# fryzjergda/DesiRNA

Hardware: AMD Instinct MI355X
Metric: replica-folds/sec (MFE+PF, L=200, R=64) (higher is better)
Workload: dtype int32 (MFE) + f64 (PF); 1 GPU; BASELINE configs[2]: Eterna100-V1 #69 target (L=200), R=64 uniform-random sequences per GPU, -sf Ed-Epf (MFE fill+traceback, PF inside, eval_structure); replicas_per_gpu=64, replicas_total=64, replicas_on_rank0=64, L=200, exchange_every=100, threads_per_workgroup=1024

## Files before the change

desirna_amd/csrc/fold_pf_lds.hpp:

```cpp
#pragma once
#include <cstddef>
#include "eval_structure.hpp"
#include "fold_pf.hpp"

namespace drna {

constexpr int PF_FAST_NMAX = 200;
constexpr int PGSLOTS = 10;
constexpr int PNG = 3;
constexpr int TSL = 14;

template <int NT>
struct PfFastSmem {
  static constexpr int NW = NT / WAVE;
  static constexpr int RS = PF_FAST_NMAX + 2;
  static constexpr int NSLOT = 4 * WAVE;
  static constexpr int NL = PF_FAST_NMAX + 8;
  double qbi[32 * RS];
  double dring[4 * RS];
  double qm1row[2][RS];
  double urow[2][RS];
  double hpw[PF_FAST_NMAX + 2];
  double q5[PF_FAST_NMAX + 2];
  double partG[2][2][NSLOT];
  double partK[2][4][NSLOT];
  double accE[2][NSLOT], accX[2][3][NSLOT];
  double stack[64], mmH[128], mmI[128], mm1n[128], mm23[128], mmM[128], mmExt[128], int11[1024], d5[32], d3[32];
  double rinv[128];
  double rbul[128];
  double r1n[128];
  double r23[128];
  double eWt[36][2];
  double xc[16];
  double twc[32][2];
  int plist[2][NL];
  int pcnt[2];
  int qhead[2];
  int qtile[2];
  unsigned char info[32 * RS];
  unsigned char S[PF_FAST_NMAX + 4];
  int flag;
};

template <int NT>
__device__ __forceinline__ void pf_q5_column(PfFastSmem<NT>& sm, const double* __restrict__ QEXT, int ld, int j, int lane,
                                             double sc1) {
  double s = 0.0;
  for (int i = lane + 1; i <= j - TURN - 1; i += WAVE) s += sm.q5[i - 1] * QEXT[j * ld + i];
  s = wave_total_f64_lane63(s);
  if (lane == WAVE - 1) sm.q5[j] = sm.q5[j - 1] * sc1 + s;
  wave_lds_sync();
}

template <class SM>
__device__ __forceinline__ void pf_prepare_tables(SM& sm, int d, int tid) {
  constexpr int RS = SM::RS;
  if (tid >= 0 && tid < GRES) {
    const int par = d & 1;
    const int x = (int)((unsigned)(d + 50 - tid) % (unsigned)GRES);
    const int zero_row = 32 * RS * 8;
    int offA = zero_row, offB = zero_row;
    double eas = 0.0, keep = 1.0, W = 0.0;
    if (x <= 26) {
      const int s = x + 4, dp = d - 6 - x;
      if (dp <= TURN) keep = 0.0;
      else {
        const int base = (dp & 31) * RS * 8;
        offA = base + 3 * 8;
        offB = s == 4 ? zero_row : base + (s - 1) * 8;
        eas = sm.tw_as[s];
        keep = s <= 5 ? 0.0 : 1.0;
        W = sm.tw_W[s];
      }
    }
    sm.tw_i[par][tid][0] = offA; sm.tw_i[par][tid][1] = offB;
    sm.tw_d[par][tid][0] = eas; sm.tw_d[par][tid][1] = keep; sm.tw_d[par][tid][2] = W;
  }
}

__device__ __forceinline__ double lane_table_f64(double v, int l) {
  return __hiloint2double(__builtin_amdgcn_readlane(__double2hiint(v), l), __builtin_amdgcn_readlane(__double2loint(v), l));
}

template <class SM, int R0, int R1>
__device__ __forceinline__ double pf_tower_part(const SM& sm, double (&G)[PGSLOTS], int i8, int eA, int eB, double eas,
                                                double ekeep, double eW) {
  const char* ring = reinterpret_cast<const char*>(sm.qbi);
  double a[R1 - R0], b[R1 - R0];
#pragma unroll
  for (int r = R0; r < R1; r++) {
    a[r - R0] = *reinterpret_cast<const double*>(ring + lane_table(eA, r) + i8);
    b[r - R0] = *reinterpret_cast<const double*>(ring + lane_table(eB, r) + i8);
  }
  double acc = 0.0;
#pragma unroll
  for (int r = R0; r < R1; r++) {
    G[r] = G[r] * lane_table_f64(ekeep, r) + (a[r - R0] + b[r - R0]) * lane_table_f64(eas, r);
    acc += G[r] * lane_table_f64(eW, r);
  }
  return acc;
}

template <class SM>
__device__ __forceinline__ double pf_tower_step(const SM& sm, double (&G)[PGSLOTS], int par, int i8, int g, int lane) {
  const int rr = lane * PNG + g;
  const bool on = lane < PGSLOTS && rr < GRES;
  const int zero_row = 32 * SM::RS * 8;
  const int eA = on ? sm.tw_i[par][rr][0] : zero_row, eB = on ? sm.tw_i[par][rr][1] : zero_row;
  const double eas = on ? sm.tw_d[par][rr][0] : 0.0, ekeep = on ? sm.tw_d[par][rr][1] : 1.0, eW = on ? sm.tw_d[par][rr][2] : 0.0;
  const double lo = pf_tower_part<SM, 0, PGSLOTS / 2>(sm, G, i8, eA, eB, eas, ekeep, eW);
  const double hi = pf_tower_part<SM, PGSLOTS / 2, PGSLOTS>(sm, G, i8, eA, eB, eas, ekeep, eW);
  return lo + hi;
}


template <class SM, int SIG, int Q0, int Q1>
__device__ __forceinline__ void pf_tower2_part(const SM& sm, double (&G)[TSL], int dv, int i8, int cbase, double& acc) {
  const char* ring = reinterpret_cast<const char*>(sm.qbi);
  double a[Q1 - Q0], b[Q1 - Q0];
  f64x2 c[Q1 - Q0];
#pragma unroll
  for (int q = Q1 - 1; q >= Q0; q--) {
    const int s = 4 + SIG + 2 * q;
    if (s > 30) continue;
    const int va = ((dv - s) & 31) * (SM::RS * 8) + i8;
    a[q - Q0] = *reinterpret_cast<const double*>(ring + va + 24);
    b[q - Q0] = s == 4 ? 0.0 : *reinterpret_cast<const double*>(ring + va + (s - 1) * 8);
    c[q - Q0] = *reinterpret_cast<const f64x2*>(ring + cbase + s * 16);
  }
#pragma unroll
  for (int q = Q1 - 1; q >= Q0; q--) {
    const int s = 4 + SIG + 2 * q;
    if (s > 30) continue;
    G[q] = q > 0 ? fma3_f64(a[q - Q0] + b[q - Q0], c[q - Q0].x, G[q - 1]) : (a[q - Q0] + b[q - Q0]) * c[q - Q0].x;
    acc += G[q] * c[q - Q0].y;
  }
}

template <class SM, int SIG>
__device__ __forceinline__ double pf_tower2_step(const SM& sm, double (&G)[TSL], int dv, int i8) {
  const int cbase = as_vector((int)(reinterpret_cast<const char*>(&sm.twc[0][0]) - reinterpret_cast<const char*>(sm.qbi)));
  double acc0 = 0.0, acc1 = 0.0, acc2 = 0.0;
  pf_tower2_part<SM, SIG, 9, 14>(sm, G, dv, i8, cbase, acc0);
  pf_tower2_part<SM, SIG, 4, 9>(sm, G, dv, i8, cbase, acc1);
  pf_tower2_part<SM, SIG, 0, 4>(sm, G, dv, i8, cbase, acc2);
  return (acc0 + acc1) + acc2;
}


#ifndef DRNA_PKE
#define DRNA_PKE 5
#endif
constexpr int PKE = DRNA_PKE;
constexpr int KT_NL = PKE + 3;
constexpr int KT_U = (2 * KT_NL + 3) / 4;
constexpr int KT_BMIN = (12 + 2 * PKE + 3) / 4;
constexpr int KT_D0 = 4 * KT_BMIN - 3;
constexpr int KT_MF = (4 * ((PF_FAST_NMAX - 1) / 4) - 11 - 2 * PKE + 15) / 16;
constexpr int KT_DEPTH = 3;
static_assert(PKE >= 4, "a tile's operands must be final when the first of its four steps comes");

__device__ __forceinline__ void kt_near_counts(int i, int d, int& nl, int& nh) {
  const int j = i + d, a = (i - 1) >> 2, c = (j - 1) >> 2, tot = max(d - 2 * TURN - 2, 0);
  if (c - a >= KT_BMIN) { nl = 4 * a + 4 + PKE - i; nh = j - 4 * c - 1 + PKE; }
  else { nl = min(tot, KT_NL); nh = tot - nl; }
}
__device__ __forceinline__ bool kt_has_far(int i, int d) { return ((i + d - 1) >> 2) - ((i - 1) >> 2) >= KT_BMIN; }

template <typename RS>
__device__ __forceinline__ void k_near_row(RS rs, int tab8, int ld, int d, int i, int row, double& v0, double& v1) {
  int nl0, nh0, nl1, nh1;
  kt_near_counts(i, d, nl0, nh0);
  kt_near_counts(i + 1, d, nl1, nh1);
  f64x2 a[KT_U], c[KT_U];
#pragma unroll
  for (int u = 0; u < KT_U; u++) {
    const int s = row + 4 * u, y = s - KT_NL;
    const bool low = s < KT_NL;
    const bool ok0 = low ? s < nl0 : y < nh0, ok1 = low ? s < nl1 : y < nh1;
    int tt = low ? TURN + 1 + s : d - TURN - 2 - y;
    tt = (ok0 || ok1) ? tt : TURN + 1;
    a[u] = buf_load_f64x2(rs, (tt * ld + i) * 8, 0);
    c[u] = buf_load_f64x2(rs, tab8 + ((d - tt - 1) * ld + i + tt + 1) * 8, 0);
    if (!ok0) a[u].x = 0.0;
    if (!ok1) a[u].y = 0.0;
  }
  double p0 = 0.0, p1 = 0.0, q0 = 0.0, q1 = 0.0;
#pragma unroll
  for (int u = 0; u < KT_U; u++) {
    if (u & 1) { p1 = fma(a[u].x, c[u].x, p1); q1 = fma(a[u].y, c[u].y, q1); }
    else { p0 = fma(a[u].x, c[u].x, p0); q0 = fma(a[u].y, c[u].y, q0); }
  }
  v0 = p0 + p1; v1 = q0 + q1;
}

constexpr int KT_PRE = 3;
struct KTile {
  double al, bl, av[KT_PRE], bv[KT_PRE];
  int vA, vB;
  int a, c, last;
  bool mask_last;
};
template <bool SC1, typename RS>
__device__ __forceinline__ void k_tile_issue(RS rs, int tab8, int ld, int n, int a, int B, int lane, KTile& t) {
  const int c = a + B, m_lo = 4 * a + 9 + PKE, m_hi = 4 * c - 3 - PKE;
  const int last = __builtin_amdgcn_readfirstlane((m_hi - m_lo + 16) >> 4) - 1;
  const int q = lane & 3, moff = (lane & 12) + (lane >> 4);
  const int i = 4 * a + 1 + q, jc = min(4 * c + 1 + q, n);
  const int sA = 16 * ld * 8, sB = 16 * (ld - 1) * 8;
  const int m0 = m_lo + moff, ml = min(m0 + 16 * last, m_hi);
  const int vA = (i - (1 + i) * ld + m0 * ld) * 8;
  const int vB = tab8 + (jc * ld - (m0 + 16 * last) * (ld - 1)) * 8;
  const int vAl = (i - (1 + i) * ld + ml * ld) * 8, vBl = tab8 + (jc * ld - ml * (ld - 1)) * 8;
  t.a = a; t.c = c; t.last = last; t.mask_last = m0 + 16 * last > m_hi; t.vA = vA; t.vB = vB;
#pragma unroll
  for (int u = 0; u < KT_PRE; u++) {
    if (u < last) {
      t.av[u] = SC1 ? buf_load_f64_aux(rs, vA, u * sA) : buf_load_f64(rs, vA, u * sA);
      t.bv[u] = SC1 ? buf_load_f64_aux(rs, vB, (last - u) * sB) : buf_load_f64(rs, vB, (last - u) * sB);
    }
  }
  t.al = SC1 ? buf_load_f64_aux(rs, vAl, 0) : buf_load_f64(rs, vAl, 0);
  t.bl = SC1 ? buf_load_f64_aux(rs, vBl, 0) : buf_load_f64(rs, vBl, 0);
}
template <bool SC1, typename RS, typename ST>
__device__ __forceinline__ void k_tile_finish(RS rs, int ld, const KTile& t, int n, int lane, ST store) {
  const int sA = 16 * ld * 8, sB = 16 * (ld - 1) * 8, last = t.last;
  double acc0 = 0.0, acc1 = 0.0;
#pragma unroll
  for (int u = 0; u < KT_PRE; u++) {
    if (u < last) {
      if (u & 1) acc1 = mfma_f64_4x4x4_4b(t.av[u], t.bv[u], acc1);
      else acc0 = mfma_f64_4x4x4_4b(t.av[u], t.bv[u], acc0);
    }
  }
#pragma unroll
  for (int u0 = KT_PRE; u0 < KT_MF - 1; u0 += KT_DEPTH) {
    if (u0 < last) {
      double av[KT_DEPTH], bv[KT_DEPTH];
#pragma unroll
      for (int w = 0; w < KT_DEPTH; w++) {
        const int u = u0 + w;
        if (u < last && u < KT_MF - 1) {
          av[w] = SC1 ? buf_load_f64_aux(rs, t.vA, u * sA) : buf_load_f64(rs, t.vA, u * sA);
          bv[w] = SC1 ? buf_load_f64_aux(rs, t.vB, (last - u) * sB) : buf_load_f64(rs, t.vB, (last - u) * sB);
        }
      }
#pragma unroll
      for (int w = 0; w < KT_DEPTH; w++) {
        const int u = u0 + w;
        if (u < last && u < KT_MF - 1) {
          if (u & 1) acc1 = mfma_f64_4x4x4_4b(av[w], bv[w], acc1);
          else acc0 = mfma_f64_4x4x4_4b(av[w], bv[w], acc0);
        }
      }
    }
  }
  const double al = t.mask_last ? 0.0 : t.al;
  if (last & 1) acc1 = mfma_f64_4x4x4_4b(al, t.bl, acc1);
  else acc0 = mfma_f64_4x4x4_4b(al, t.bl, acc0);
  double v = acc0 + acc1;
  v = dpp_add_f64<0x114, 0xF>(v);
  v = dpp_add_f64<0x118, 0xF>(v);
  const int ii = 4 * t.a + 1 + (lane >> 4), jj = 4 * t.c + 1 + (lane & 3);
  if ((lane & 12) == 12 && jj <= n) store(jj - ii, ii, v);
}

#ifndef DRNA_PFL_D1
#define DRNA_PFL_D1 24
#endif
constexpr int PFL_D1 = DRNA_PFL_D1;
template <bool AGENT, class SM>
__device__ __forceinline__ void pf_pl_row(const SM& sm, int32_t* PL, int ld, int n, int d, int lane) {
  int cntb = 0;
  for (int i0 = 1; i0 <= n - d; i0 += WAVE) {
    const int i = i0 + lane;
    int t = 0;
    if (i <= n - d) t = pair_type(sm.S[i], sm.S[i + d]);
    const unsigned long long m = __ballot(t != 0);
    if (t) {
      const int pos = cntb + __popcll(m & ((1ull << lane) - 1ull));
      const int32_t w = i | ((t * 16 + sm.S[i + 1] * 4 + sm.S[i + d - 1]) << 8);
      if (AGENT) st_agent(&PL[d * ld + pos], w); else PL[d * ld + pos] = w;
    }
    cntb += __popcll(m);
  }
  if (lane == 0) { if (AGENT) st_agent(&PL[d * ld + ld - 1], (int32_t)cntb); else PL[d * ld + ld - 1] = cntb; }
}

template <int NT>
__device__ __forceinline__ void pf_kfar_helper(const PfArgs& A, const EvalArgs& EV, PfFastSmem<NT>& sm, int r, int n) {
  constexpr int NW = NT / WAVE;
  const int ld = A.ld, tid = threadIdx.x, lane = lane_id();
  const int wave = __builtin_amdgcn_readfirstlane(wave_id());
  double* base = A.ws + (long long)r * A.ws_stride;
  const long long tab = (long long)ld * ld;
  double* DFAR = base + 5 * tab;
  const auto rsX = __builtin_amdgcn_make_buffer_rsrc((void*)base, (short)0, (int)(2 * tab * 8), 0x00020000);
  const int* flagA = A.hflags + (long long)r * 64;
  int* flagB = A.hflags + (long long)r * 64 + 32;
  int* ctl = reinterpret_cast<int*>(&sm);
  if (tid == 0) ctl[0] = 0;
  if (EV.n_targets > 0) {
    constexpr int NEV = NW < 8 ? NW : 8;
    EvalSmem* es = reinterpret_cast<EvalSmem*>(ctl + 32);
    if (wave < NEV)
      for (int k = wave; k < EV.n_targets; k += NEV) eval_one(es[wave], EV, r, k, lane);
  }
  {
    const char* seq = A.seqs + A.rg.off_of(r, n);
    for (int k = tid; k < n; k += NT) { const int c = enc_nt(seq[k]); sm.S[k + 1] = (unsigned char)(c < 0 ? 0 : c); }
    if (tid == 0) { sm.S[0] = 0; sm.S[n + 1] = 0; }
    __syncthreads();
    int32_t* PL = reinterpret_cast<int32_t*>(base + 4 * tab);
    for (int d = PFL_D1 + wave; d < n; d += NW) pf_pl_row<true>(sm, PL, ld, n, d, lane);
    drain_vmem();
  }
  __syncthreads();
  if (tid == 0) st_agent(flagB, A.hbase + KT_D0 - 1);
  const int Bmax = (n - 1) >> 2;
  for (int B = KT_BMIN; B <= Bmax; B++) {
    if (wave == 0) {
      int seen = 0;
      const bool ok = strip_wait(flagA, A.hbase, 4 * B - 5 - PKE, seen);
      if (lane == 0 && (!ok || seen == A.hbase + STRIP_DONE)) ctl[0] = 1;
    }
    __syncthreads();
    if (ctl[0]) break;
    if (!(DRNA_SKIP & 8))
      for (int a = wave; a <= Bmax - B; a += NW) {
        KTile t;
        k_tile_issue<true>(rsX, (int)tab * 8, ld, n, a, B, lane, t);
        k_tile_finish<true>(rsX, ld, t, n, lane, [&](int d, int i, double v) { st_agent(&DFAR[d * ld + i], v); });
      }
    drain_vmem();
    __syncthreads();
    if (tid == 0) st_agent(flagB, A.hbase + (B == Bmax ? n : 4 * B));
  }
}

template <int NT, bool TILES = true>
__device__ __forceinline__ void pf_lds_body(PfFastSmem<NT>& sm, PfArgs A, const EvalArgs& EV, int bx_in = -1, int helper_in = -1) {
  constexpr int NW = NT / WAVE;
  constexpr int RS = PfFastSmem<NT>::RS;
  const PfTables& T = *A.T;
  const bool hm = A.helper != 0;
  const int bx = bx_in >= 0 ? bx_in : hm ? blockIdx.x >> 1 : blockIdx.x;
  const bool is_helper = hm && (helper_in >= 0 ? helper_in != 0 : (blockIdx.x & 1) != 0);
  const int r = A.rg.seq_of(bx);
  A.L = A.rg.len_of(r, A.L);
  const int n = A.L, ld = A.ld;
  if (is_helper) {
    if (A.helper == 2) return;
    pf_kfar_helper<NT>(A, EV, sm, r, n);
    return;
  }
  const int tid = threadIdx.x, lane = lane_id();
  const int wave = __builtin_amdgcn_readfirstlane(wave_id());

  double* base = A.ws + (long long)r * A.ws_stride;
  const long long tab = (long long)ld * ld;
  double* QM = base + 2 * tab;
  double* QM1 = base + 3 * tab;
  int32_t* PL = reinterpret_cast<int32_t*>(base + 4 * tab);
  double* QEXT = base + 6 * tab;

  const double eTau = T.TermAU, eMLc = T.MLclosing, eMLi = T.MLintern;
  const double b1 = A.eMLb[1], sc1 = A.scale[1], sc2 = A.scale[2];

  stage_energy_tables<NT>(sm, T, tid);
  for (int k = tid; k < 128; k += NT) {
    const double inv = 1.0 / T.mmI[k];
    sm.rinv[k] = inv;
    sm.rbul[k] = ((k >> 4) > 2 ? eTau : 1.0) * inv;
    sm.r1n[k] = T.mm1n[k] * inv;
    sm.r23[k] = T.mm23[k] * inv;
  }
  for (int k = tid; k <= n; k += NT) sm.hpw[k] = A.hp_w[k];
  for (int t = tid; t < 36; t += NT) {
    sm.eWt[t][0] = t >= 2 && t <= 30 ? T.bulge[t] * A.scale[t + 2] : 0.0;
    sm.eWt[t][1] = t >= 4 && t <= 30 ? T.interior[t] * T.eninio[t - 2] * A.scale[t + 2] : 0.0;
  }
  if (tid == 0) {
    sm.xc[0] = T.bulge[1] * A.scale[3]; sm.xc[1] = T.interior[5] * T.eninio[1] * A.scale[7];
    sm.xc[2] = A.scale[4]; sm.xc[3] = A.scale[5]; sm.xc[4] = A.scale[6];
    sm.xc[8] = eTau; sm.xc[9] = eMLc; sm.xc[10] = eMLi; sm.xc[11] = b1; sm.xc[12] = sc2;
  }
  for (int k = tid; k < 32; k += NT) {
    sm.twc[k][0] = k >= 4 && k <= 30 ? T.eninio[k - 4] : 0.0;
    sm.twc[k][1] = k >= 6 && k <= 30 ? T.interior[k] * A.scale[k + 2] : 0.0;
  }
  for (int k = tid; k < 4 * RS; k += NT) sm.dring[k] = 0.0;
  for (int k = tid; k < 32 * RS; k += NT) { sm.qbi[k] = 0.0; sm.info[k] = 0; }
  for (int k = tid; k < 2 * RS; k += NT) { (&sm.qm1row[0][0])[k] = 0.0; (&sm.urow[0][0])[k] = 0.0; }
  for (int k = tid; k < 2 * 2 * PfFastSmem<NT>::NSLOT; k += NT) (&sm.partG[0][0][0])[k] = 0.0;
  for (int k = tid; k < 2 * 4 * PfFastSmem<NT>::NSLOT; k += NT) (&sm.partK[0][0][0])[k] = 0.0;
  for (int k = tid; k < 2 * PfFastSmem<NT>::NSLOT; k += NT) (&sm.accE[0][0])[k] = 0.0;
  for (int k = tid; k < 6 * PfFastSmem<NT>::NSLOT; k += NT) (&sm.accX[0][0][0])[k] = 0.0;
  if (tid == 0) sm.q5[0] = 1.0;
  load_sequence<NT>(sm, A.seqs + A.rg.off_of(r, n), n, tid);
  if (sm.flag) {
    if (tid == 0) { A.status[r] = ST_BAD_CHAR; A.Epf[r] = 0.0; if (hm) st_agent(A.hflags + (long long)r * 64, A.hbase + STRIP_DONE); }
    return;
  }
  if (wave == 0) {
    for (int j = 1; j <= n && j <= TURN + 1; j++) sm.q5[j] = sm.q5[j - 1] * sc1;
  }
  for (int d = TURN + 1 + wave; d < (hm ? min(n, PFL_D1) : n); d += NW) pf_pl_row<false>(sm, PL, ld, n, d, lane);
  __syncthreads();

  const int NB = (n + WAVE - 1) / WAVE;
  const int off0 = (NB * WAVE - n) / 2;
  const int aw = wave - NB;
  constexpr bool TWO_PAR = NT < 1024;
  const int nT = n - 10, NBT = nT > 0 ? (nT + WAVE - 1) / WAVE : 0;
  const int T0 = max(0, off0 + 5 - (NBT * WAVE - nT) / 2);
  int my_tb = -1, my_sig = 0, my_pm = 0;
  if (aw >= 0) {
    if (TWO_PAR) { if (aw < 2 * NBT) { my_tb = aw >> 1; my_sig = aw & 1; my_pm = 3; } }
    else if (aw < 4 * NBT) { my_tb = aw >> 2; const int x = (aw + my_tb) & 3; my_sig = x & 1; my_pm = 1 << (x >> 1); }
  }
  const int w_pl = NB > 2 ? 2 : 0, w_q5 = NB - 1;

  if (aw < 0) {
    const int d = TURN + 1;
    if (d < n) {
      const int cnt = PL[d * ld + ld - 1];
      if (tid < cnt) sm.plist[d & 1][tid] = PL[d * ld + tid];
      if (tid == 0) { sm.pcnt[d & 1] = cnt; sm.qhead[0] = 0; sm.qhead[1] = 0; sm.qtile[0] = 0; sm.qtile[1] = 0; }
    }
  }
  __syncthreads();


  const auto rsQ = __builtin_amdgcn_make_buffer_rsrc((void*)QM, (short)0, (int)(2 * tab * 8), 0x00020000);


  double* XQM = base, *XQM1 = base + tab, *DFAR = base + 5 * tab;
  int* flagA = hm ? A.hflags + (long long)r * 64 : nullptr;
  const int* flagB = hm ? A.hflags + (long long)r * 64 + 32 : nullptr;
  double dfar_cur = 0.0, dfar_next = 0.0;
  int fb_last = 0;
  bool helper_lost = false, pl_seen = false;
  auto run_items = [&](const int d) {
    const int ncell = n - d, sh = d >> 1, par = d & 1;
    const int slot0 = sh + off0 - 1;
    const int pcnt = __builtin_amdgcn_readfirstlane(sm.pcnt[par]);
    const int nblk = (ncell + 31) >> 5;
    const int nK = ((DRNA_SKIP & 8) || d < 2 * TURN + 3) ? 0 : nblk;
    const int nE = (DRNA_SKIP & 2) ? 0 : (pcnt + 3) >> 2, nX = (DRNA_SKIP & 4) ? 0 : 3 * ((pcnt + WAVE - 1) / WAVE);
    const int nItems = __builtin_amdgcn_readfirstlane(nK + nE + nX);
    for (int it0 = queue_pop(&sm.qhead[par], lane); it0 < nItems; it0 = queue_pop(&sm.qhead[par], lane)) {
      const int it = it0 < nX ? nK + nE + it0 : it0 - nX;
      if (it < nK) {
        const int blk = it, cl = lane & 15, row = lane >> 4;
        int i = (blk << 5) + 2 * cl + 1;
        const bool act0 = i <= ncell, act1 = i + 1 <= ncell;
        i = act0 ? i : 1;
        double v0, v1;
        k_near_row(rsQ, (int)tab * 8, ld, d, i, row, v0, v1);
        if (act0) sm.partK[par][row][i + slot0] = v0;
        if (act1) sm.partK[par][row][i + 1 + slot0] = v1;
      } else if (it < nK + nE) {
        const int q = 4 * (it - nK) + (lane >> 4);
        const int pe = sm.plist[par][q < pcnt ? q : pcnt - 1];
        const int i0 = pe & 255, ij = pe >> 8;
        const int tA = (lane & 15) + 2, tBr = tA + 16, tB = tBr > 30 ? 30 : tBr;
        const f64x2 wA = *reinterpret_cast<const f64x2*>(&sm.eWt[tA][0]), wB = *reinterpret_cast<const f64x2*>(&sm.eWt[tBr][0]);
        const int oA = ((d - 2 - tA) & 31) * RS + i0, oB = ((d - 2 - tB) & 31) * RS + i0;
        const double a1 = sm.qbi[oA + 1], a2 = sm.qbi[oA + 2], a3 = sm.qbi[oA + tA], a4 = sm.qbi[oA + tA + 1];
        const double b1_ = sm.qbi[oB + 1], b2_ = sm.qbi[oB + 2], b3_ = sm.qbi[oB + tB], b4_ = sm.qbi[oB + tB + 1];
        const int fa1 = sm.info[oA + 1], fa2 = sm.info[oA + 2], fa3 = sm.info[oA + tA], fa4 = sm.info[oA + tA + 1];
        const int fb1 = sm.info[oB + 1], fb2 = sm.info[oB + 2], fb3 = sm.info[oB + tB], fb4 = sm.info[oB + tB + 1];
        const double ra1 = sm.rbul[fa1], ra4 = sm.rbul[fa4], ra2 = sm.r1n[fa2], ra3 = sm.r1n[fa3];
        const double rb1 = sm.rbul[fb1], rb4 = sm.rbul[fb4], rb2 = sm.r1n[fb2], rb3 = sm.r1n[fb3];
        const double bul = (a1 * ra1 + a4 * ra4) * wA.x + (b1_ * rb1 + b4_ * rb4) * wB.x;
        const double one = (a2 * ra2 + a3 * ra3) * wA.y + (b2_ * rb2 + b3_ * rb3) * wB.y;
        double v = bul * ((ij >> 4) > 2 ? sm.xc[as_vector(8)] : 1.0) + one * sm.mm1n[ij];
        v = dpp_add_f64<0x111, 0xF>(v);
        v = dpp_add_f64<0x112, 0xF>(v);
        v = dpp_add_f64<0x114, 0xF>(v);
        v = dpp_add_f64<0x118, 0xF>(v);
        if ((lane & 15) == 15 && q < pcnt) sm.accE[par][i0 + slot0] = v;
      } else {
        const int xi = it - nK - nE;
        const int ch = xi / 3, grp = xi - 3 * ch;
        const int q = ch * WAVE + lane;
        const int pe = sm.plist[par][q < pcnt ? q : pcnt - 1];
        const int i = pe & 255, cxv = pe >> 8, t = cxv >> 4, si1 = (cxv >> 2) & 3, sj1 = cxv & 3;
        double sum;
        if (grp == 0) {
          double w[4];
          int f[4];
#pragma unroll
          for (int shp = 0; shp < 4; shp++) {
            const int u1 = shp >> 1, u2 = shp == 1 || shp == 3 ? 1 : 0;
            const int dp = d - 2 - u1 - u2;
            const int off = (dp & 31) * RS + 1 + u1 + i;
            w[shp] = dp > TURN ? sm.qbi[off] : 0.0;
            f[shp] = dp > TURN ? sm.info[off] : 0;
          }
          sum = w[0] * sm.rinv[f[0]] * sm.stack[t * 8 + (f[0] >> 4)] * sm.xc[as_vector(12)];
          sum += (w[1] * sm.rinv[f[1]] * sm.stack[t * 8 + (f[1] >> 4)] + w[2] * sm.rinv[f[2]] * sm.stack[t * 8 + (f[2] >> 4)]) * sm.xc[as_vector(0)];
          sum += w[3] * sm.rinv[f[3]] * sm.int11[(t * 8 + (f[3] >> 4)) * 16 + si1 * 4 + sj1] * sm.xc[as_vector(2)];
        } else if (grp == 1) {
          const int dpa = d - 5, dpb = d - 6;
          const int oa = (dpa & 31) * RS + 2 + i, ob = (dpa & 31) * RS + 3 + i, oc = (dpb & 31) * RS + 3 + i;
          const double wa = dpa > TURN ? sm.qbi[oa] : 0.0, wb = dpa > TURN ? sm.qbi[ob] : 0.0, wc = dpb > TURN ? sm.qbi[oc] : 0.0;
          const int fa = dpa > TURN ? sm.info[oa] : 0, fb = dpa > TURN ? sm.info[ob] : 0, fc = dpb > TURN ? sm.info[oc] : 0;
          const double ga = T.int21[(t * 8 + (fa >> 4)) * 64 + si1 * 16 + ((fa >> 2) & 3) * 4 + sj1];
          const double gb = T.int21[((fb >> 4) * 8 + t) * 64 + ((fb >> 2) & 3) * 16 + si1 * 4 + (fb & 3)];
          const double gc = T.int22[(t * 8 + (fc >> 4)) * 256 + si1 * 64 + (fc & 3) * 16 + ((fc >> 2) & 3) * 4 + sj1];
          sum = (wa * sm.rinv[fa] * ga + wb * sm.rinv[fb] * gb) * sm.xc[as_vector(3)] + wc * sm.rinv[fc] * gc * sm.xc[as_vector(4)];
        } else {
          const int dp = d - 7;
          const int oa = (dp & 31) * RS + 3 + i, ob = (dp & 31) * RS + 4 + i;
          const double wa = dp > TURN ? sm.qbi[oa] : 0.0, wb = dp > TURN ? sm.qbi[ob] : 0.0;
          const int fa = dp > TURN ? sm.info[oa] : 0, fb = dp > TURN ? sm.info[ob] : 0;
          sum = (wa * sm.r23[fa] + wb * sm.r23[fb]) * sm.mm23[cxv] * sm.xc[as_vector(1)];
        }
        if (q < pcnt) sm.accX[par][grp][i + slot0] = sum;
      }
    }
  };

  auto run_tiles = [&](const int d) {
    const int Bmax = (n - 1) >> 2, Bt = ((d + 3) >> 2) + 1, ph = (d + 3) & 3;
    if (!TILES || (DRNA_SKIP & 8) || hm || Bt < KT_BMIN || Bt > Bmax) return;
    const int cnt = Bmax - Bt + 1, per = (cnt + 3) >> 2, a0 = ph * per;
    const int nT = __builtin_amdgcn_readfirstlane(max(0, min(cnt, a0 + per) - a0));
    for (int it = queue_pop(&sm.qtile[d & 1], lane); it < nT; it = queue_pop(&sm.qtile[d & 1], lane)) {
      KTile t;
      k_tile_issue<false>(rsQ, (int)tab * 8, ld, n, a0 + it, Bt, lane, t);
      k_tile_finish<false>(rsQ, ld, t, n, lane, [&](int dd, int ii, double v) { DFAR[dd * ld + ii] = v; });
    }
  };

  if (aw < 0) {
    double fTau = sm.xc[as_vector(8)], fMLc = sm.xc[as_vector(9)], fMLi = sm.xc[as_vector(10)], fb1 = sm.xc[as_vector(11)], fsc2 = sm.xc[as_vector(12)];
    int pl_cnt = 0, pl0 = 0, pl1 = 0, pl2 = 0, pl3 = 0;
    auto pl_request = [&](const int dn) {
      const int32_t* row = PL + dn * ld;
      if (hm && dn >= PFL_D1) {
        if (!pl_seen) {
          int seen = 0;
          if (!helper_lost && !flag_ge(fb_last, A.hbase + KT_D0 - 1) && !strip_wait(flagB, A.hbase, KT_D0 - 1, seen)) { sm.flag = 2; helper_lost = true; }
          pl_seen = true;
        }
        pl_cnt = ld_agent(row + ld - 1);
        pl0 = ld_agent(row + lane); pl1 = ld_agent(row + lane + WAVE); pl2 = ld_agent(row + lane + 2 * WAVE);
        pl3 = ld_agent(row + min(lane + 3 * WAVE, ld - 1));
      } else {
        pl_cnt = row[ld - 1];
        pl0 = row[lane]; pl1 = row[lane + WAVE]; pl2 = row[lane + 2 * WAVE]; pl3 = row[min(lane + 3 * WAVE, ld - 1)];
      }
    };
    if (wave == w_pl && TURN + 2 < n) pl_request(TURN + 2);
    for (int k = TURN + 1; k <= n; k++) {
      const int d = k - 1;
      if (wave == w_pl) {
        if (k + 1 < n) {
          int* dst = sm.plist[(k + 1) & 1];
          dst[lane] = pl0; dst[lane + WAVE] = pl1; dst[lane + 2 * WAVE] = pl2;
          if (lane + 3 * WAVE < PfFastSmem<NT>::NL) dst[lane + 3 * WAVE] = pl3;
          if (lane == 0) { sm.pcnt[(k + 1) & 1] = pl_cnt; sm.qhead[(k + 1) & 1] = 0; sm.qtile[(k + 1) & 1] = 0; }
        }
        if (k + 2 < n) pl_request(k + 2);
      }
      const bool job_q5 = wave == w_q5 && k - 3 >= TURN + 2;
      double qx0 = 0.0, qx1 = 0.0, qx2 = 0.0, qx3 = 0.0;
      if (job_q5) {
        const int j = k - 3, top = j - TURN - 1;
        const double* col = QEXT + j * ld;
        qx0 = lane + 1 <= top ? col[lane + 1] : 0.0;
        qx1 = lane + 1 + WAVE <= top ? col[lane + 1 + WAVE] : 0.0;
        qx2 = lane + 1 + 2 * WAVE <= top ? col[lane + 1 + 2 * WAVE] : 0.0;
        qx3 = lane + 1 + 3 * WAVE <= top ? col[lane + 1 + 3 * WAVE] : 0.0;
      }
      int f_req = 0;
      double d_req = 0.0;
      dfar_cur = dfar_next;
      if (hm) {
        if (tid == 0 && k - 2 > TURN) st_agent(flagA, A.hbase + (k - 2));
        f_req = ld_agent(flagB);
        if (k >= KT_D0 && k < n && !helper_lost && !flag_ge(fb_last, A.hbase + k)) {
          int seen = 0;
          if (!strip_wait(flagB, A.hbase, k, seen)) { sm.flag = 2; helper_lost = true; }
        }
      }
      if (k >= KT_D0 && k < n) {
        const int ic = tid + 1 - (k >> 1) - off0;
        if (ic >= 1 && ic <= n - k && kt_has_far(ic, k)) d_req = hm ? ld_agent(&DFAR[k * ld + ic]) : DFAR[k * ld + ic];
      }
      if (d > TURN) {
        const int ncell = n - d, sh = d >> 1, par = d & 1;
        const int i = tid + 1 - sh - off0;
        if (i >= 1 && i <= ncell) {
          const int j = i + d;
          const int si = sm.S[i], sj = sm.S[j], si1 = sm.S[i + 1],
                    sj1 = sm.S[j - 1], sim = sm.S[i - 1], sjp = sm.S[j + 1];
          const double aG = d >= 10 ? sm.partG[par][0][tid] + sm.partG[par][1][tid] : 0.0;
          const double aKn = d >= 2 * TURN + 3 ? (sm.partK[par][0][tid] + sm.partK[par][1][tid]) + (sm.partK[par][2][tid] + sm.partK[par][3][tid]) : 0.0;
          const double aK = aKn + dfar_cur;
          const int t = pair_type(si, sj);
          const double cTau = fTau, cMLc = fMLc, cMLi = fMLi, cb1 = fb1, csc2 = fsc2;
          const double tau = t > 2 ? cTau : 1.0;
          const int ij = t * 16 + si1 * 4 + sj1, rt = rtype_of(t);
          const int info = t ? (rt << 4) | (sjp << 2) | sim : 0;
          const double aE = sm.accE[par][tid], aX = (sm.accX[par][0][tid] + sm.accX[par][1][tid]) + sm.accX[par][2][tid];
          const double wH = sm.mmH[ij], wI = sm.mmI[ij], wMc = sm.mmM[rt * 16 + sj1 * 4 + si1], wInfo = sm.mmI[info];
          const double dprev = sm.dring[((d - 2) & 3) * RS + i + 1];
          const int ex = t * 16 + sim * 4 + sjp;
          const double wExt = sm.mmExt[ex], wMs = sm.mmM[ex], w5 = sm.d5[t * 4 + sim], w3 = sm.d3[t * 4 + sjp];
          const int pp = (d - 1) & 1;
          const double m1p = sm.qm1row[pp][i], m1q = sm.qm1row[pp][i + 1], up = sm.urow[pp][i + 1];
          double qb = 0.0;
          if (t) {
            const int u = d - 1;
            double hp;
            if (u == 3 || u == 4 || u == 6) {
              int code = 0;
              const int len = u + 2;
              for (int q = 0; q < len; q++) code |= sm.S[i + q] << (2 * q);
              hp = -1.0;
              if (u == 3) { for (int q = 0; q < T.n_tri; q++) if (T.tri_code[q] == code) hp = T.tri_w[q] * A.scale[u + 2]; if (hp < 0.0) hp = sm.hpw[u] * tau; }
              else if (u == 4) { for (int q = 0; q < T.n_tetra; q++) if (T.tetra_code[q] == code) hp = T.tetra_w[q] * A.scale[u + 2]; }
              else { for (int q = 0; q < T.n_hexa; q++) if (T.hexa_code[q] == code) hp = T.hexa_w[q] * A.scale[u + 2]; }
              if (hp < 0.0) hp = sm.hpw[u] * wH;
            } else {
              hp = sm.hpw[u] * wH;
            }
            qb = hp + aE + aX + aG * wI;
            qb += dprev * cMLc * cMLi * tau * wMc * csc2;
          }
          sm.qbi[(d & 31) * RS + i] = qb * wInfo;
          sm.info[(d & 31) * RS + i] = (unsigned char)info;
          const double me = (i > 1 && j < n) ? wExt : i > 1 ? w5 : j < n ? w3 : 1.0;
          const double mm = (i > 1 && j < n) ? wMs : i > 1 ? w5 : j < n ? w3 : 1.0;
          const double ext = t ? qb * tau * me : 0.0, stem = t ? qb * cMLi * tau * mm : 0.0;
          const double m1 = m1p * cb1 + stem;
          const double U = cb1 * (m1q + up);
          sm.qm1row[par][i] = m1;
          sm.urow[par][i] = U;
          sm.dring[(d & 3) * RS + i] = aK;
          {
            QEXT[j * ld + i] = ext;
            QM1[d * ld + i] = m1;
            QM[d * ld + i] = m1 + aK + U;
            if (hm) { st_agent(&XQM1[d * ld + i], m1); st_agent(&XQM[d * ld + i], m1 + aK + U); }
          }
        }
      }
      if (job_q5) {
        const int j = k - 3, top = j - TURN - 1;
        double sq = 0.0;
        if (lane + 1 <= top) sq += sm.q5[lane] * qx0;
        if (lane + 1 + WAVE <= top) sq += sm.q5[lane + WAVE] * qx1;
        if (lane + 1 + 2 * WAVE <= top) sq += sm.q5[lane + 2 * WAVE] * qx2;
        if (lane + 1 + 3 * WAVE <= top) sq += sm.q5[lane + 3 * WAVE] * qx3;
        sq = wave_total_f64_lane63(sq);
        if (lane == WAVE - 1) sm.q5[j] = sm.q5[j - 1] * sc1 + sq;
      }
      if (k < n) run_items(k);
      dfar_next = d_req;
      if (hm) fb_last = __builtin_amdgcn_readfirstlane(f_req);
      __syncthreads();
    }
  } else {
    double GE[TSL], GO[TSL];
#pragma unroll
    for (int q = 0; q < TSL; q++) { GE[q] = 0.0; if (TWO_PAR) GO[q] = 0.0; }
    for (int k = TURN + 1; k <= n; k++) {
      if (k < n) {
        const int d = k;
        const int ncell = n - d, sh = d >> 1, par = d & 1;
        const int lo = sh + off0, hi = ncell + sh + off0 - 1;

        if (!(DRNA_SKIP & 1) && ((my_pm >> par) & 1) && d >= 10) {
          const int blo = T0 + my_tb * WAVE;
          int i = blo + lane + 1 - sh - off0;
          i = i < 1 ? 1 : (i > ncell ? ncell : i);
          const int dv = as_vector(d + 30), i8 = i * 8;
          if (blo <= hi && blo + WAVE - 1 >= lo) {
            double accG = 0.0;
            if constexpr (TWO_PAR) {
              if (par) accG = my_sig ? pf_tower2_step<PfFastSmem<NT>, 1>(sm, GO, dv, i8) : pf_tower2_step<PfFastSmem<NT>, 0>(sm, GO, dv, i8);
            }
            if (!TWO_PAR || !par) accG = my_sig ? pf_tower2_step<PfFastSmem<NT>, 1>(sm, GE, dv, i8) : pf_tower2_step<PfFastSmem<NT>, 0>(sm, GE, dv, i8);
            sm.partG[par][my_sig][T0 + my_tb * WAVE + lane] = accG;
          }
        }
        run_tiles(d);
        run_items(d);
      }
      __syncthreads();
    }
  }

  const int jq0 = max(TURN + 2, n - 2);
  if (NW >= 3) {
    if (wave < 3 && jq0 + wave <= n) {
      const int j = jq0 + wave;
      double sq = 0.0;
      for (int i = lane + 1; i <= j - TURN - 1; i += WAVE) sq += sm.q5[i - 1] * QEXT[j * ld + i];
      sq = wave_total_f64_lane63(sq);
      if (lane == WAVE - 1) sm.xc[13 + wave] = sq;
    }
    __syncthreads();
    if (tid == 0)
      for (int j = jq0; j <= n; j++) sm.q5[j] = sm.q5[j - 1] * sc1 + sm.xc[13 + j - jq0];
    __syncthreads();
  } else if (wave == 0) {
    for (int j = jq0; j <= n; j++) pf_q5_column<NT>(sm, QEXT, ld, j, lane, sc1);
  }
  if (wave == 0) {
    if (lane == 0) {
      const double Z = sm.q5[n];
      if (!(Z > 0.0) || !(Z < 1.0e300)) {
        A.status[r] = ST_PF_RANGE;
        A.Epf[r] = 0.0;
      } else {
        A.status[r] = sm.flag == 2 ? ST_SYNC : ST_OK;
        A.Epf[r] = (-log(Z) - (double)n * log(T.pf_scale)) * T.kT / 1000.0;
      }
      if (hm) st_agent(flagA, A.hbase + STRIP_DONE);
    }
  }
}

template <int NT, bool TILES = true>
__global__ __launch_bounds__(NT) void pf_lds_kernel(PfArgs A, EvalArgs EV, int R) {
  __shared__ PfFastSmem<NT> sm;
  if (!TILES && !A.helper) return;
  int bx = -1, is_helper = -1;
  if (A.helper) {
    pair_block(blockIdx.x, bx, is_helper);
    if (bx >= R) return;
  }
  pf_lds_body<NT, TILES>(sm, A, EV, bx, is_helper);
}

}
```

Measured before the change: 151,100 replica-folds/s.

## Offload far bulge/1n-interior sums to helper block and split near sums

Splits the per-diagonal bulge/interior-loop accumulation into a near part (loop sizes 2-9 or 2-17) computed in the main block, and a far part (sizes 10-30). When a helper block is active, the helper computes the far part from qb values the main block mirrors into global memory. Without a helper, the far part becomes a separate work item in the main queue. The helper also stages the bulge tables and builds pair lists in LDS ahead of each strip. This is meant to take work off the serial critical-path diagonal loop, at the cost of extra global stores and loads, agent-scope synchronization and a tighter wait condition in the helper.

```diff
diff --git a/desirna_amd/csrc/fold_pf_lds.hpp b/desirna_amd/csrc/fold_pf_lds.hpp
--- a/desirna_amd/csrc/fold_pf_lds.hpp
+++ b/desirna_amd/csrc/fold_pf_lds.hpp
@@ -25,6 +25,7 @@
   double partG[2][2][NSLOT];
   double partK[2][4][NSLOT];
   double accE[2][NSLOT], accX[2][3][NSLOT];
+  double accF[2][NSLOT];
   double stack[64], mmH[128], mmI[128], mm1n[128], mm23[128], mmM[128], mmExt[128], int11[1024], d5[32], d3[32];
   double rinv[128];
   double rbul[128];
@@ -288,6 +289,64 @@
   if (lane == 0) { if (AGENT) st_agent(&PL[d * ld + ld - 1], (int32_t)cntb); else PL[d * ld + ld - 1] = cntb; }
 }
 
+constexpr int EF_T0 = 10;
+constexpr int EF_D0 = KT_D0;
+static_assert(PKE <= 7, "a helper round's far bulge sums read rows up to 4B - 12");
+static_assert(EF_D0 - 6 <= 17, "below EF_D0 the near items cover every size with one size per lane");
+struct EfOps { double a1, a2, a3, a4, b1, b2, b3, b4; };
+__device__ __forceinline__ void ef_sizes(int lane, int& tA, int& tB, int& wB) {
+  tA = EF_T0 + (lane & 15);
+  const int tBr = tA + 16;
+  tB = tBr > 30 ? 30 : tBr;
+  wB = tBr > 35 ? 35 : tBr;
+}
+template <int NT, class SM>
+__device__ __forceinline__ void pf_stage_bulge_tables(SM& sm, const PfTables& T, const PfArgs& A, int tid) {
+  const double eTau = T.TermAU;
+  for (int k = tid; k < 128; k += NT) {
+    const double inv = 1.0 / T.mmI[k];
+    sm.rinv[k] = inv;
+    sm.rbul[k] = ((k >> 4) > 2 ? eTau : 1.0) * inv;
+    sm.r1n[k] = T.mm1n[k] * inv;
+    sm.r23[k] = T.mm23[k] * inv;
+  }
+  for (int t = tid; t < 36; t += NT) {
+    sm.eWt[t][0] = t >= 2 && t <= 30 ? T.bulge[t] * A.scale[t + 2] : 0.0;
+    sm.eWt[t][1] = t >= 4 && t <= 30 ? T.interior[t] * T.eninio[t - 2] * A.scale[t + 2] : 0.0;
+  }
+}
+template <class SM>
+__device__ __forceinline__ double pf_efar_sum(const SM& sm, const EfOps& o, int fa1, int fa2, int fa3, int fa4, int fb1, int fb2,
+                                              int fb3, int fb4, int lane, int ij) {
+  int tA, tB, wBi;
+  ef_sizes(lane, tA, tB, wBi);
+  const f64x2 wA = *reinterpret_cast<const f64x2*>(&sm.eWt[tA][0]), wB = *reinterpret_cast<const f64x2*>(&sm.eWt[wBi][0]);
+  const double bulA = fma(o.a1, sm.rbul[fa1], o.a4 * sm.rbul[fa4]), bulB = fma(o.b1, sm.rbul[fb1], o.b4 * sm.rbul[fb4]);
+  const double oneA = fma(o.a2, sm.r1n[fa2], o.a3 * sm.r1n[fa3]), oneB = fma(o.b2, sm.r1n[fb2], o.b3 * sm.r1n[fb3]);
+  const double bul = fma(bulA, wA.x, bulB * wB.x), one = fma(oneA, wA.y, oneB * wB.y);
+  double v = fma(bul, (ij >> 4) > 2 ? sm.xc[as_vector(8)] : 1.0, one * sm.mm1n[ij]);
+  v = dpp_add_f64<0x111, 0xF>(v);
+  v = dpp_add_f64<0x112, 0xF>(v);
+  v = dpp_add_f64<0x114, 0xF>(v);
+  v = dpp_add_f64<0x118, 0xF>(v);
+  return v;
+}
+__device__ __forceinline__ int ef_mirror(int ld, int d, int i) { return (ld - 1 - d) * ld + (ld - 1 - i); }
+
+template <class SM>
+__device__ __forceinline__ int pf_pl_row_lds(const SM& sm, int* row, int n, int d, int lane) {
+  int cntb = 0;
+  for (int i0 = 1; i0 <= n - d; i0 += WAVE) {
+    const int i = i0 + lane;
+    int t = 0;
+    if (i <= n - d) t = pair_type(sm.S[i], sm.S[i + d]);
+    const unsigned long long m = __ballot(t != 0);
+    if (t) row[cntb + __popcll(m & ((1ull << lane) - 1ull))] = i | ((t * 16 + sm.S[i + 1] * 4 + sm.S[i + d - 1]) << 8);
+    cntb += __popcll(m);
+  }
+  return cntb;
+}
+
 template <int NT>
 __device__ __forceinline__ void pf_kfar_helper(const PfArgs& A, const EvalArgs& EV, PfFastSmem<NT>& sm, int r, int n) {
   constexpr int NW = NT / WAVE;
@@ -296,11 +355,22 @@
   double* base = A.ws + (long long)r * A.ws_stride;
   const long long tab = (long long)ld * ld;
   double* DFAR = base + 5 * tab;
+  const double* XQB = base;
+  double* EFAR = base + 5 * tab;
   const auto rsX = __builtin_amdgcn_make_buffer_rsrc((void*)base, (short)0, (int)(2 * tab * 8), 0x00020000);
   const int* flagA = A.hflags + (long long)r * 64;
   int* flagB = A.hflags + (long long)r * 64 + 32;
   int* ctl = reinterpret_cast<int*>(&sm);
+  constexpr int HLS = 256, HLR = 8;
+  int* hcnt = ctl + 16;
+  int* hl = ctl + 64;
+  static_assert((64 + HLR * HLS) * 4 <= (int)sizeof(sm.qbi), "helper lists live in the ring");
   if (tid == 0) ctl[0] = 0;
+  if (!(DRNA_SKIP & 2)) {
+    pf_stage_bulge_tables<NT>(sm, *A.T, A, tid);
+    for (int k = tid; k < 128; k += NT) sm.mm1n[k] = A.T->mm1n[k];
+    if (tid == 0) sm.xc[8] = A.T->TermAU;
+  }
   if (EV.n_targets > 0) {
     constexpr int NEV = NW < 8 ? NW : 8;
     EvalSmem* es = reinterpret_cast<EvalSmem*>(ctl + 32);
@@ -310,7 +380,8 @@
   {
     const char* seq = A.seqs + A.rg.off_of(r, n);
     for (int k = tid; k < n; k += NT) { const int c = enc_nt(seq[k]); sm.S[k + 1] = (unsigned char)(c < 0 ? 0 : c); }
-    if (tid == 0) { sm.S[0] = 0; sm.S[n + 1] = 0; }
+    __syncthreads();
+    if (tid == 0) { sm.S[0] = sm.S[n]; sm.S[n + 1] = sm.S[1]; }
     __syncthreads();
     int32_t* PL = reinterpret_cast<int32_t*>(base + 4 * tab);
     for (int d = PFL_D1 + wave; d < n; d += NW) pf_pl_row<true>(sm, PL, ld, n, d, lane);
@@ -319,10 +390,16 @@
   __syncthreads();
   if (tid == 0) st_agent(flagB, A.hbase + KT_D0 - 1);
   const int Bmax = (n - 1) >> 2;
-  for (int B = KT_BMIN; B <= Bmax; B++) {
+  const int Bend = n > EF_D0 ? max(Bmax, KT_BMIN) : Bmax;
+  for (int B = KT_BMIN; B <= Bend; B++) {
+    const int e0 = 4 * B - 3, e1 = B == Bend ? n - 1 : 4 * B, nr = (DRNA_SKIP & 2) ? 0 : e1 - e0 + 1;
+    for (int rr = wave; rr < nr; rr += NW) {
+      const int cnt = pf_pl_row_lds(sm, hl + rr * HLS, n, e0 + rr, lane);
+      if (lane == 0) hcnt[rr] = cnt;
+    }
     if (wave == 0) {
       int seen = 0;
-      const bool ok = strip_wait(flagA, A.hbase, 4 * B - 5 - PKE, seen);
+      const bool ok = strip_wait(flagA, A.hbase, max(4 * B - 5 - PKE, e1 - 2 - EF_T0), seen);
       if (lane == 0 && (!ok || seen == A.hbase + STRIP_DONE)) ctl[0] = 1;
     }
     __syncthreads();
@@ -333,9 +410,55 @@
         k_tile_issue<true>(rsX, (int)tab * 8, ld, n, a, B, lane, t);
         k_tile_finish<true>(rsX, ld, t, n, lane, [&](int d, int i, double v) { st_agent(&DFAR[d * ld + i], v); });
       }
+    {
+      int tot = 0;
+      for (int rr = 0; rr < nr; rr++) tot += (hcnt[rr] + 3) >> 2;
+      tot = __builtin_amdgcn_readfirstlane(tot);
+      auto ef_load = [&](int it, int& dI, int& pe, bool& ok, EfOps& o) {
+        int rr = 0;
+        for (; rr < nr - 1; rr++) { const int c = (hcnt[rr] + 3) >> 2; if (it < c) break; it -= c; }
+        rr = __builtin_amdgcn_readfirstlane(rr);
+        const int cnt = hcnt[rr], q = 4 * it + (lane >> 4);
+        dI = e0 + rr; ok = q < cnt; pe = hl[rr * HLS + (ok ? q : cnt - 1)];
+        const int i0 = pe & 255;
+        int tA, tB, wBi;
+        ef_sizes(lane, tA, tB, wBi);
+        const int dA = dI - 2 - tA, dB = dI - 2 - tB;
+        const bool hA = dA > TURN, hB = dB > TURN;
+        const int mA = ef_mirror(ld, hA ? dA : TURN + 1, i0), mB = ef_mirror(ld, hB ? dB : TURN + 1, i0);
+        o.a1 = ld_agent(&XQB[mA - 1]); o.a2 = ld_agent(&XQB[mA - 2]); o.a3 = ld_agent(&XQB[mA - tA]); o.a4 = ld_agent(&XQB[mA - tA - 1]);
+        o.b1 = ld_agent(&XQB[mB - 1]); o.b2 = ld_agent(&XQB[mB - 2]); o.b3 = ld_agent(&XQB[mB - tB]); o.b4 = ld_agent(&XQB[mB - tB - 1]);
+        if (!hA) { o.a1 = 0.0; o.a2 = 0.0; o.a3 = 0.0; o.a4 = 0.0; }
+        if (!hB) { o.b1 = 0.0; o.b2 = 0.0; o.b3 = 0.0; o.b4 = 0.0; }
+      };
+      auto info_of = [&](int dp, int p) {
+        if (dp <= TURN) return 0;
+        const int q = p + dp, t = pair_type(sm.S[p], sm.S[q]);
+        return t ? (rtype_of(t) << 4) | (sm.S[q + 1] << 2) | sm.S[p - 1] : 0;
+      };
+      auto ef_finish = [&](int dI, int pe, bool ok, const EfOps& o) {
+        const int i0 = pe & 255;
+        int tA, tB, wBi;
+        ef_sizes(lane, tA, tB, wBi);
+        const int dA = dI - 2 - tA, dB = dI - 2 - tB;
+        const double v = pf_efar_sum(sm, o, info_of(dA, i0 + 1), info_of(dA, i0 + 2), info_of(dA, i0 + tA), info_of(dA, i0 + tA + 1),
+                                     info_of(dB, i0 + 1), info_of(dB, i0 + 2), info_of(dB, i0 + tB), info_of(dB, i0 + tB + 1), lane, pe >> 8);
+        if ((lane & 15) == 15 && ok) st_agent(&EFAR[ef_mirror(ld, dI, i0)], v);
+      };
+      for (int it = wave; it < tot; it += 2 * NW) {
+        int d0, p0, d1 = 0, p1 = 0;
+        bool k0, k1 = false;
+        EfOps o0, o1;
+        const bool two = it + NW < tot;
+        ef_load(it, d0, p0, k0, o0);
+        if (two) ef_load(it + NW, d1, p1, k1, o1);
+        ef_finish(d0, p0, k0, o0);
+        if (two) ef_finish(d1, p1, k1, o1);
+      }
+    }
     drain_vmem();
     __syncthreads();
-    if (tid == 0) st_agent(flagB, A.hbase + (B == Bmax ? n : 4 * B));
+    if (tid == 0) st_agent(flagB, A.hbase + (B == Bend ? n : 4 * B));
   }
 }
 
@@ -369,18 +492,8 @@
   const double b1 = A.eMLb[1], sc1 = A.scale[1], sc2 = A.scale[2];
 
   stage_energy_tables<NT>(sm, T, tid);
-  for (int k = tid; k < 128; k += NT) {
-    const double inv = 1.0 / T.mmI[k];
-    sm.rinv[k] = inv;
-    sm.rbul[k] = ((k >> 4) > 2 ? eTau : 1.0) * inv;
-    sm.r1n[k] = T.mm1n[k] * inv;
-    sm.r23[k] = T.mm23[k] * inv;
-  }
+  pf_stage_bulge_tables<NT>(sm, T, A, tid);
   for (int k = tid; k <= n; k += NT) sm.hpw[k] = A.hp_w[k];
-  for (int t = tid; t < 36; t += NT) {
-    sm.eWt[t][0] = t >= 2 && t <= 30 ? T.bulge[t] * A.scale[t + 2] : 0.0;
-    sm.eWt[t][1] = t >= 4 && t <= 30 ? T.interior[t] * T.eninio[t - 2] * A.scale[t + 2] : 0.0;
-  }
   if (tid == 0) {
     sm.xc[0] = T.bulge[1] * A.scale[3]; sm.xc[1] = T.interior[5] * T.eninio[1] * A.scale[7];
     sm.xc[2] = A.scale[4]; sm.xc[3] = A.scale[5]; sm.xc[4] = A.scale[6];
@@ -395,7 +508,7 @@
   for (int k = tid; k < 2 * RS; k += NT) { (&sm.qm1row[0][0])[k] = 0.0; (&sm.urow[0][0])[k] = 0.0; }
   for (int k = tid; k < 2 * 2 * PfFastSmem<NT>::NSLOT; k += NT) (&sm.partG[0][0][0])[k] = 0.0;
   for (int k = tid; k < 2 * 4 * PfFastSmem<NT>::NSLOT; k += NT) (&sm.partK[0][0][0])[k] = 0.0;
-  for (int k = tid; k < 2 * PfFastSmem<NT>::NSLOT; k += NT) (&sm.accE[0][0])[k] = 0.0;
+  for (int k = tid; k < 2 * PfFastSmem<NT>::NSLOT; k += NT) { (&sm.accE[0][0])[k] = 0.0; (&sm.accF[0][0])[k] = 0.0; }
   for (int k = tid; k < 6 * PfFastSmem<NT>::NSLOT; k += NT) (&sm.accX[0][0][0])[k] = 0.0;
   if (tid == 0) sm.q5[0] = 1.0;
   load_sequence<NT>(sm, A.seqs + A.rg.off_of(r, n), n, tid);
@@ -437,9 +550,11 @@
 
 
   double* XQM = base, *XQM1 = base + tab, *DFAR = base + 5 * tab;
+  double* XQB = base;
+  const double* EFAR = base + 5 * tab;
   int* flagA = hm ? A.hflags + (long long)r * 64 : nullptr;
   const int* flagB = hm ? A.hflags + (long long)r * 64 + 32 : nullptr;
-  double dfar_cur = 0.0, dfar_next = 0.0;
+  double dfar_cur = 0.0, dfar_next = 0.0, efar_cur = 0.0, efar_next = 0.0;
   int fb_last = 0;
   bool helper_lost = false, pl_seen = false;
   auto run_items = [&](const int d) {
@@ -448,10 +563,12 @@
     const int pcnt = __builtin_amdgcn_readfirstlane(sm.pcnt[par]);
     const int nblk = (ncell + 31) >> 5;
     const int nK = ((DRNA_SKIP & 8) || d < 2 * TURN + 3) ? 0 : nblk;
-    const int nE = (DRNA_SKIP & 2) ? 0 : (pcnt + 3) >> 2, nX = (DRNA_SKIP & 4) ? 0 : 3 * ((pcnt + WAVE - 1) / WAVE);
-    const int nItems = __builtin_amdgcn_readfirstlane(nK + nE + nX);
+    const int elw = d < EF_D0 ? 4 : 3, ecl = 6 - elw;
+    const int nE = (DRNA_SKIP & 2) ? 0 : (pcnt + (1 << ecl) - 1) >> ecl, nX = (DRNA_SKIP & 4) ? 0 : 3 * ((pcnt + WAVE - 1) / WAVE);
+    const int nF = (!TILES || hm || (DRNA_SKIP & 2) || d < EF_D0) ? 0 : (pcnt + 3) >> 2;
+    const int nItems = __builtin_amdgcn_readfirstlane(nK + nE + nF + nX);
     for (int it0 = queue_pop(&sm.qhead[par], lane); it0 < nItems; it0 = queue_pop(&sm.qhead[par], lane)) {
-      const int it = it0 < nX ? nK + nE + it0 : it0 - nX;
+      const int it = it0 < nX ? nK + nE + nF + it0 : it0 - nX;
       if (it < nK) {
         const int blk = it, cl = lane & 15, row = lane >> 4;
         int i = (blk << 5) + 2 * cl + 1;
@@ -462,28 +579,39 @@
         if (act0) sm.partK[par][row][i + slot0] = v0;
         if (act1) sm.partK[par][row][i + 1 + slot0] = v1;
       } else if (it < nK + nE) {
-        const int q = 4 * (it - nK) + (lane >> 4);
+        const int q = ((it - nK) << ecl) + (lane >> elw), el = lane & ((1 << elw) - 1);
         const int pe = sm.plist[par][q < pcnt ? q : pcnt - 1];
         const int i0 = pe & 255, ij = pe >> 8;
-        const int tA = (lane & 15) + 2, tBr = tA + 16, tB = tBr > 30 ? 30 : tBr;
-        const f64x2 wA = *reinterpret_cast<const f64x2*>(&sm.eWt[tA][0]), wB = *reinterpret_cast<const f64x2*>(&sm.eWt[tBr][0]);
-        const int oA = ((d - 2 - tA) & 31) * RS + i0, oB = ((d - 2 - tB) & 31) * RS + i0;
+        const int tA = el + 2;
+        const f64x2 wA = *reinterpret_cast<const f64x2*>(&sm.eWt[tA][0]);
+        const int oA = ((d - 2 - tA) & 31) * RS + i0;
         const double a1 = sm.qbi[oA + 1], a2 = sm.qbi[oA + 2], a3 = sm.qbi[oA + tA], a4 = sm.qbi[oA + tA + 1];
-        const double b1_ = sm.qbi[oB + 1], b2_ = sm.qbi[oB + 2], b3_ = sm.qbi[oB + tB], b4_ = sm.qbi[oB + tB + 1];
         const int fa1 = sm.info[oA + 1], fa2 = sm.info[oA + 2], fa3 = sm.info[oA + tA], fa4 = sm.info[oA + tA + 1];
-        const int fb1 = sm.info[oB + 1], fb2 = sm.info[oB + 2], fb3 = sm.info[oB + tB], fb4 = sm.info[oB + tB + 1];
-        const double ra1 = sm.rbul[fa1], ra4 = sm.rbul[fa4], ra2 = sm.r1n[fa2], ra3 = sm.r1n[fa3];
-        const double rb1 = sm.rbul[fb1], rb4 = sm.rbul[fb4], rb2 = sm.r1n[fb2], rb3 = sm.r1n[fb3];
-        const double bul = (a1 * ra1 + a4 * ra4) * wA.x + (b1_ * rb1 + b4_ * rb4) * wB.x;
-        const double one = (a2 * ra2 + a3 * ra3) * wA.y + (b2_ * rb2 + b3_ * rb3) * wB.y;
-        double v = bul * ((ij >> 4) > 2 ? sm.xc[as_vector(8)] : 1.0) + one * sm.mm1n[ij];
+        const double bul = fma(a1, sm.rbul[fa1], a4 * sm.rbul[fa4]) * wA.x;
+        const double one = fma(a2, sm.r1n[fa2], a3 * sm.r1n[fa3]) * wA.y;
+        double v = fma(bul, (ij >> 4) > 2 ? sm.xc[as_vector(8)] : 1.0, one * sm.mm1n[ij]);
         v = dpp_add_f64<0x111, 0xF>(v);
         v = dpp_add_f64<0x112, 0xF>(v);
         v = dpp_add_f64<0x114, 0xF>(v);
-        v = dpp_add_f64<0x118, 0xF>(v);
-        if ((lane & 15) == 15 && q < pcnt) sm.accE[par][i0 + slot0] = v;
+        if (elw == 4) v = dpp_add_f64<0x118, 0xF>(v);
+        if (el == (1 << elw) - 1 && q < pcnt) sm.accE[par][i0 + slot0] = v;
+      } else if (it < nK + nE + nF) {
+        if constexpr (TILES) {
+          const int q = 4 * (it - nK - nE) + (lane >> 4);
+          const int pe = sm.plist[par][q < pcnt ? q : pcnt - 1];
+          const int i0 = pe & 255;
+          int tA, tB, wBi;
+          ef_sizes(lane, tA, tB, wBi);
+          const int oA = ((d - 2 - tA) & 31) * RS + i0, oB = ((d - 2 - tB) & 31) * RS + i0;
+          EfOps o;
+          o.a1 = sm.qbi[oA + 1]; o.a2 = sm.qbi[oA + 2]; o.a3 = sm.qbi[oA + tA]; o.a4 = sm.qbi[oA + tA + 1];
+          o.b1 = sm.qbi[oB + 1]; o.b2 = sm.qbi[oB + 2]; o.b3 = sm.qbi[oB + tB]; o.b4 = sm.qbi[oB + tB + 1];
+          const double v = pf_efar_sum(sm, o, sm.info[oA + 1], sm.info[oA + 2], sm.info[oA + tA], sm.info[oA + tA + 1],
+                                       sm.info[oB + 1], sm.info[oB + 2], sm.info[oB + tB], sm.info[oB + tB + 1], lane, pe >> 8);
+          if ((lane & 15) == 15 && q < pcnt) sm.accF[par][i0 + slot0] = v;
+        }
       } else {
-        const int xi = it - nK - nE;
+        const int xi = it - nK - nE - nF;
         const int ch = xi / 3, grp = xi - 3 * ch;
         const int q = ch * WAVE + lane;
         const int pe = sm.plist[par][q < pcnt ? q : pcnt - 1];
@@ -578,8 +706,9 @@
         qx3 = lane + 1 + 3 * WAVE <= top ? col[lane + 1 + 3 * WAVE] : 0.0;
       }
       int f_req = 0;
-      double d_req = 0.0;
+      double d_req = 0.0, e_req = 0.0;
       dfar_cur = dfar_next;
+      efar_cur = efar_next;
       if (hm) {
         if (tid == 0 && k - 2 > TURN) st_agent(flagA, A.hbase + (k - 2));
         f_req = ld_agent(flagB);
@@ -591,6 +720,7 @@
       if (k >= KT_D0 && k < n) {
         const int ic = tid + 1 - (k >> 1) - off0;
         if (ic >= 1 && ic <= n - k && kt_has_far(ic, k)) d_req = hm ? ld_agent(&DFAR[k * ld + ic]) : DFAR[k * ld + ic];
+        if (hm && ic >= 1 && ic <= n - k) e_req = ld_agent(&EFAR[ef_mirror(ld, k, ic)]);
       }
       if (d > TURN) {
         const int ncell = n - d, sh = d >> 1, par = d & 1;
@@ -607,7 +737,8 @@
           const double tau = t > 2 ? cTau : 1.0;
           const int ij = t * 16 + si1 * 4 + sj1, rt = rtype_of(t);
           const int info = t ? (rt << 4) | (sjp << 2) | sim : 0;
-          const double aE = sm.accE[par][tid], aX = (sm.accX[par][0][tid] + sm.accX[par][1][tid]) + sm.accX[par][2][tid];
+          const double aEf = d < EF_D0 ? 0.0 : hm ? efar_cur : TILES ? sm.accF[par][tid] : 0.0;
+          const double aE = sm.accE[par][tid] + aEf, aX = (sm.accX[par][0][tid] + sm.accX[par][1][tid]) + sm.accX[par][2][tid];
           const double wH = sm.mmH[ij], wI = sm.mmI[ij], wMc = sm.mmM[rt * 16 + sj1 * 4 + si1], wInfo = sm.mmI[info];
           const double dprev = sm.dring[((d - 2) & 3) * RS + i + 1];
           const int ex = t * 16 + sim * 4 + sjp;
@@ -647,7 +778,7 @@
             QEXT[j * ld + i] = ext;
             QM1[d * ld + i] = m1;
             QM[d * ld + i] = m1 + aK + U;
-            if (hm) { st_agent(&XQM1[d * ld + i], m1); st_agent(&XQM[d * ld + i], m1 + aK + U); }
+            if (hm) { st_agent(&XQM1[d * ld + i], m1); st_agent(&XQM[d * ld + i], m1 + aK + U); st_agent(&XQB[ef_mirror(ld, d, i)], qb * wInfo); }
           }
         }
       }
@@ -663,6 +794,7 @@
       }
       if (k < n) run_items(k);
       dfar_next = d_req;
+      efar_next = e_req;
       if (hm) fb_last = __builtin_amdgcn_readfirstlane(f_req);
       __syncthreads();
     }
```

New measurement: 102,700 replica-folds/s. 0.68x the previous value.
